# marja-w/gan-des-midi-music-gen

Hardware: AMD Instinct MI355X
Metric: GAN training samples/sec (G+D step) (higher is better)
Workload: dtype bf16; 1 GPU; SIMNN G/D iteration, synthetic 128x256 spectrogram windows; per_gpu_batch=256, global_batch=256, mode=faithful, parallelism=dp1

## Files before the change

### gan_des_midi_music_gen_amd/csrc/gemm_bf16.hip

```cpp
#include "gemm_common.h"

namespace {

constexpr int BM = 128, BN = 128;

inline bool operand_ok(const void* p, int dtype, int64_t s_row, int64_t s_k, int rows, int K, bool* kmaj) {
  const int64_t esz = dtype == GDM_BF16 ? 2 : 4, epc = 16 / esz;
  if (((uintptr_t)p & 15) != 0) return false;
  if (s_k == 1 && s_row >= 1 && (s_row * esz) % 16 == 0 && K % epc == 0) {
    *kmaj = true;
    return ((int64_t)(rows - 1) * s_row + K) * esz < ((int64_t)1 << 31);
  }
  if (s_row == 1 && s_k >= 1 && (s_k * esz) % 16 == 0 && rows % epc == 0) {
    *kmaj = false;
    return ((int64_t)(K - 1) * s_k + rows) * esz < ((int64_t)1 << 31);
  }
  return false;
}

}

bool gdm_gemm_bf16_fast_ok(const GemmArgs& g, int a_dtype, int b_dtype, bool* a_kmaj, bool* b_kmaj) {
  if (!operand_ok(g.A, a_dtype, g.sam, g.sak, g.M, g.K, a_kmaj)) return false;
  if (!operand_ok(g.B, b_dtype, g.sbn, g.sbk, g.N, g.K, b_kmaj)) return false;
  if (g.scn != 1) return false;
  const int64_t csz = g.c_dtype == GDM_BF16 ? 2 : 4;
  if (g.N % 4 == 0) {
    if ((g.scm * csz) % (4 * csz) != 0 || ((uintptr_t)g.C & (4 * csz - 1)) != 0) return false;
    if (g.bias_n && ((uintptr_t)g.bias_n & 15) != 0) return false;
  }
  if ((int64_t)g.M * g.N < 64 * 64) return false;
  return true;
}

bool gdm_gemm_bf16_fast_deep(int M, int N, int split_k, int k_per_split) {
  const int MT = (M + BM - 1) / BM, NTl = (N + BN - 1) / BN;
  const int outer = NTl * split_k;
  bool deep = split_k > 1 && (int64_t)outer * MT <= 512 && k_per_split >= 256;
  static const int force = GDM_TUNABLE("GDM_GEMM_VARIANT", -1);
  if (force >= 0) deep = force == 1;
  return deep;
}

int gdm_gemm_bf16_fast_launch(const GemmArgs& g, int a_dtype, int b_dtype, const GemmPlan& p, hipStream_t s) {
  const int MT = (g.M + BM - 1) / BM, NTl = (g.N + BN - 1) / BN;
  const int outer = NTl * g.split_k;
  dim3 grid((unsigned)(((outer + 7) / 8) * 8 * MT));
  const bool deep = p.kernel == GDM_GEMM_KERNEL_FAST_K64;
  auto* launch = a_dtype == GDM_BF16 ? (deep ? gdm_gemm_bf16_kt64_bf16a : gdm_gemm_bf16_kt32_bf16a)
                                     : (deep ? gdm_gemm_bf16_kt64_f32a : gdm_gemm_bf16_kt32_f32a);
  launch(g, p.a_kmaj, b_dtype, p.b_kmaj, grid, s);
  GDM_LAUNCH_OK("gdm_gemm(bf16 fast path)");
  return GDM_OK;
}
```

### gan_des_midi_music_gen_amd/csrc/gemm_bf16_kernel.h

```cpp
#pragma once
#include <type_traits>
#include "buffer_ops.h"
#include "gemm_common.h"

namespace {

constexpr int BM = 128, BN = 128, NT = 256;

__device__ __forceinline__ void wave_lds_sync() {
  __builtin_amdgcn_fence(__ATOMIC_RELEASE, "wavefront");
  __builtin_amdgcn_wave_barrier();
  __builtin_amdgcn_fence(__ATOMIC_ACQUIRE, "wavefront");
}

template <int ACT> __device__ __forceinline__ float act_const(float v, float slope) {
  if constexpr (ACT == GDM_ACT_RELU) return v > 0.f ? v : 0.f;
  else if constexpr (ACT == GDM_ACT_LEAKY) return v > 0.f ? v : v * slope;
  else if constexpr (ACT == GDM_ACT_SIGMOID) return 1.0f / (1.0f + expf(-v));
  else return v;
}

template <int KT> __device__ __forceinline__ int kswz(int row) { return KT == 64 ? ((row >> 1) & 7) : ((row >> 1) & 2); }
__device__ __forceinline__ int rswz(int k) { return (k & 3) | ((k >> 1) & 4); }

template <typename T, int KT> struct Stage {
  static constexpr int N = 128 * KT * (int)sizeof(T) / 16 / NT;
  f32x4 v[N];
};

template <typename T, int KT> struct Lane {
  uint32_t off[Stage<T, KT>::N];
  int kl[Stage<T, KT>::N];
  int lds[Stage<T, KT>::N];
};

template <typename T, int KT, bool KMAJ>
__device__ __forceinline__ void lane_init(Lane<T, KT>& ln, int64_t ld, int rows, int r0) {
  constexpr int EPC = 16 / sizeof(T);
  const int t = threadIdx.x;
#pragma unroll
  for (int i = 0; i < Stage<T, KT>::N; ++i) {
    const int c = t + NT * i;
    int rl, kl;
    if constexpr (KMAJ) {
      constexpr int CPR = KT / EPC;
      rl = c / CPR; kl = (c % CPR) * EPC;
      ln.off[i] = (uint32_t)(((int64_t)(r0 + rl) * ld + kl) * (int64_t)sizeof(T));
      ln.lds[i] = rl * KT + 8 * ((kl >> 3) ^ kswz<KT>(rl)) + (kl & 7);
    } else {
      constexpr int CPK = 128 / EPC;
      kl = c / CPK; rl = (c % CPK) * EPC;
      ln.off[i] = (uint32_t)(((int64_t)kl * ld + r0 + rl) * (int64_t)sizeof(T));
      ln.lds[i] = kl * 128 + (rl ^ (16 * rswz(kl)));
    }
    ln.kl[i] = (r0 + rl < rows) ? kl : -1;
  }
}

template <typename T, int KT, bool KMAJ>
__device__ __forceinline__ void stage_load(Stage<T, KT>& st, const Lane<T, KT>& ln, rsrc_t rs, int64_t ld, int k0,
                                           int kend) {
  const uint32_t kbytes = (uint32_t)((KMAJ ? (int64_t)k0 : (int64_t)k0 * ld) * (int64_t)sizeof(T));
#pragma unroll
  for (int i = 0; i < Stage<T, KT>::N; ++i) {
    const bool ok = ln.kl[i] >= 0 && k0 + ln.kl[i] < kend;
    st.v[i] = __builtin_bit_cast(f32x4, __builtin_amdgcn_raw_buffer_load_b128(rs, ok ? kbytes + ln.off[i] : BUF_OOB, 0, 0));
  }
}

template <typename T, int KT>
__device__ __forceinline__ void stage_store(const Stage<T, KT>& st, const Lane<T, KT>& ln, __bf16* __restrict__ img) {
#pragma unroll
  for (int i = 0; i < Stage<T, KT>::N; ++i) {
    if constexpr (sizeof(T) == 2) {
      *(f32x4*)(img + ln.lds[i]) = st.v[i];
    } else {
      bf16x4 h;
#pragma unroll
      for (int e = 0; e < 4; ++e) h[e] = (__bf16)st.v[i][e];
      *(bf16x4*)(img + ln.lds[i]) = h;
    }
  }
}

template <int KT, bool KMAJ>
__device__ __forceinline__ bf16x8 frag_read(const __bf16* __restrict__ img, int row0, int kk, int lr, int lg) {
  if constexpr (KMAJ) {
    const int row = row0 + lr;
    return *(const bf16x8*)&img[row * KT + 8 * ((4 * kk + lg) ^ kswz<KT>(row))];
  } else {
    const int q = lr >> 2, p = lr & 3;
    const int kr = 32 * kk + 8 * lg + q;
    const int n = (row0 + 4 * p) ^ (16 * (q | (4 * (lg & 1))));
    const bf16x4 lo = lds_tr16(&img[kr * 128 + n]);
    const bf16x4 hi = lds_tr16(&img[(kr + 4) * 128 + n]);
    return __builtin_shufflevector(lo, hi, 0, 1, 2, 3, 4, 5, 6, 7);
  }
}

template <typename TA, bool A_KMAJ, typename TB, bool B_KMAJ, int KT, int DEPTH>
__global__ __launch_bounds__(NT) void gemm_bf16_fast(GemmArgs g) {
  constexpr int IMG = 128 * KT;
  __shared__ __attribute__((aligned(16))) __bf16 smem[2 * DEPTH * IMG];
  const int t = threadIdx.x, l = t & 63, w = t >> 6, wm = w >> 1, wn = w & 1;
  const int lr = l & 15, lg = l >> 4;
  const int MT = (g.M + BM - 1) / BM, NTl = (g.N + BN - 1) / BN;
  const int id = blockIdx.x;
  const int grp = id / (8 * MT), within = id % (8 * MT);
  const int outer = grp * 8 + (within & 7), mt = within >> 3;
  if (outer >= NTl * g.split_k) return;
  const int nt = outer % NTl, zs = outer / NTl;
  const int m0 = mt * BM, n0 = nt * BN;
  const int kstep = KT * g.split_k;
  const int kbeg = zs * KT;
  const int kend = g.K;
  const int64_t lda = A_KMAJ ? g.sam : g.sak;
  const int64_t ldb = B_KMAJ ? g.sbn : g.sbk;
  const rsrc_t ra = make_rsrc(g.A, (uint32_t)((A_KMAJ ? (int64_t)(g.M - 1) * lda + g.K : (int64_t)(g.K - 1) * lda + g.M) *
                                             (int64_t)sizeof(TA)));
  const rsrc_t rb = make_rsrc(g.B, (uint32_t)((B_KMAJ ? (int64_t)(g.N - 1) * ldb + g.K : (int64_t)(g.K - 1) * ldb + g.N) *
                                             (int64_t)sizeof(TB)));
  Lane<TA, KT> la;
  Lane<TB, KT> lb;
  lane_init<TA, KT, A_KMAJ>(la, lda, g.M, m0);
  lane_init<TB, KT, B_KMAJ>(lb, ldb, g.N, n0);

  f32x4 acc[4][4];
#pragma unroll
  for (int i = 0; i < 4; ++i)
#pragma unroll
    for (int j = 0; j < 4; ++j) acc[i][j] = (f32x4){0.f, 0.f, 0.f, 0.f};

  auto multiply = [&](const __bf16* As, const __bf16* Bs) {
#pragma unroll
    for (int kk = 0; kk < KT / 32; ++kk) {
      bf16x8 a[4], b[4];
#pragma unroll
      for (int i = 0; i < 4; ++i) a[i] = frag_read<KT, A_KMAJ>(As, wm * 64 + 16 * i, kk, lr, lg);
#pragma unroll
      for (int j = 0; j < 4; ++j) b[j] = frag_read<KT, B_KMAJ>(Bs, wn * 64 + 16 * j, kk, lr, lg);
#pragma unroll
      for (int i = 0; i < 4; ++i)
#pragma unroll
        for (int j = 0; j < 4; ++j) acc[i][j] = mfma16(b[j], a[i], acc[i][j]);
    }
  };
  Stage<TA, KT> sa[DEPTH];
  Stage<TB, KT> sb[DEPTH];
  if constexpr (DEPTH == 2) {
    auto tile = [&](Stage<TA, KT>& xa, Stage<TB, KT>& xb, __bf16* As, int k0) {
      __bf16* Bs = As + IMG;
      stage_store<TA, KT>(xa, la, As);
      stage_store<TB, KT>(xb, lb, Bs);
      __syncthreads();
      stage_load<TA, KT, A_KMAJ>(xa, la, ra, lda, k0 + 2 * kstep, kend);
      stage_load<TB, KT, B_KMAJ>(xb, lb, rb, ldb, k0 + 2 * kstep, kend);
      multiply(As, Bs);
    };
    stage_load<TA, KT, A_KMAJ>(sa[0], la, ra, lda, kbeg, kend);
    stage_load<TB, KT, B_KMAJ>(sb[0], lb, rb, ldb, kbeg, kend);
    stage_load<TA, KT, A_KMAJ>(sa[1], la, ra, lda, kbeg + kstep, kend);
    stage_load<TB, KT, B_KMAJ>(sb[1], lb, rb, ldb, kbeg + kstep, kend);
    for (int k0 = kbeg; k0 < kend; k0 += 2 * kstep) {
      tile(sa[0], sb[0], smem, k0);
      tile(sa[DEPTH - 1], sb[DEPTH - 1], smem + 2 * IMG * (DEPTH - 1), k0 + kstep);
    }
  } else {
    __bf16* As = smem;
    __bf16* Bs = smem + IMG;
    stage_load<TA, KT, A_KMAJ>(sa[0], la, ra, lda, kbeg, kend);
    stage_load<TB, KT, B_KMAJ>(sb[0], lb, rb, ldb, kbeg, kend);
    for (int k0 = kbeg; k0 < kend; k0 += kstep) {
      __syncthreads();
      stage_store<TA, KT>(sa[0], la, As);
      stage_store<TB, KT>(sb[0], lb, Bs);
      __syncthreads();
      stage_load<TA, KT, A_KMAJ>(sa[0], la, ra, lda, k0 + kstep, kend);
      stage_load<TB, KT, B_KMAJ>(sb[0], lb, rb, ldb, k0 + kstep, kend);
      multiply(As, Bs);
    }
  }

  auto epilogue = [&](auto act_tag) {
    constexpr int ACT = decltype(act_tag)::value;
    const bool vec_ok = (g.N % 4 == 0);
    if (g.split_k > 1) {
#pragma unroll
      for (int i = 0; i < 4; ++i) {
        const int m = m0 + wm * 64 + 16 * i + lr;
        if (m >= g.M) continue;
#pragma unroll
        for (int j = 0; j < 4; ++j) {
          const int n = n0 + wn * 64 + 16 * j + 4 * lg;
          if (n >= g.N) continue;
          float* dst = g.ws + ((int64_t)zs * g.M + m) * g.N + n;
#ifndef GDM_GEMM_DEFAULT_STORES
          if (vec_ok) __builtin_nontemporal_store(acc[i][j], (f32x4*)dst);
#else
          if (vec_ok) *(f32x4*)dst = acc[i][j];
#endif
          else
            for (int r = 0; r < 4 && n + r < g.N; ++r) dst[r] = acc[i][j][r];
        }
      }
      return;
    }
    if (vec_ok && m0 + BM <= g.M && n0 + BN <= g.N &&
        (g.c_dtype != GDM_BF16 || (g.scm % 8 == 0 && ((uintptr_t)g.C & 15) == 0))) {
      __syncthreads();
      float* scr = (float*)smem + w * (16 * 64);
      const bool is_bf16 = g.c_dtype == GDM_BF16;
      const int prow = is_bf16 ? (l >> 3) : (l >> 4), pcol = is_bf16 ? 8 * (l & 7) : 4 * (l & 15);
      const int nn = n0 + wn * 64 + pcol;
      f32x4 bn0 = {0.f, 0.f, 0.f, 0.f}, bn1 = bn0;
      if (g.bias_n) {
        bn0 = *(const f32x4*)(g.bias_n + nn);
        if (is_bf16) bn1 = *(const f32x4*)(g.bias_n + nn + 4);
      }
      const bool has_bias = g.bias_n || g.bias_m;
#pragma unroll
      for (int i = 0; i < 4; ++i) {
        wave_lds_sync();
#pragma unroll
        for (int j = 0; j < 4; ++j) *(f32x4*)&scr[lr * 64 + 4 * ((4 * j + lg) ^ lr)] = acc[i][j];
        wave_lds_sync();
        if (is_bf16) {
#pragma unroll
          for (int h = 0; h < 2; ++h) {
            const int row = 8 * h + prow, c8 = l & 7;
            f32x4 v0 = *(const f32x4*)&scr[row * 64 + 4 * ((2 * c8) ^ row)];
            f32x4 v1 = *(const f32x4*)&scr[row * 64 + 4 * ((2 * c8 + 1) ^ row)];
            const int m = m0 + wm * 64 + 16 * i + row;
            if (has_bias) {
              const float bm = g.bias_m ? g.bias_m[m] : 0.f;
              v0 += bn0 + (f32x4){bm, bm, bm, bm};
              v1 += bn1 + (f32x4){bm, bm, bm, bm};
            }
            bf16x8 hv;
#pragma unroll
            for (int r = 0; r < 4; ++r) {
              hv[r] = (__bf16)act_const<ACT>(v0[r], g.slope);
              hv[4 + r] = (__bf16)act_const<ACT>(v1[r], g.slope);
            }
#ifndef GDM_GEMM_DEFAULT_STORES
            __builtin_nontemporal_store(hv, (bf16x8*)((__bf16*)g.C + (int64_t)m * g.scm + nn));
#else
            *(bf16x8*)((__bf16*)g.C + (int64_t)m * g.scm + nn) = hv;
#endif
          }
        } else {
#pragma unroll
          for (int h = 0; h < 4; ++h) {
            const int row = 4 * h + prow, pc = l & 15;
            f32x4 v = *(const f32x4*)&scr[row * 64 + 4 * (pc ^ row)];
            const int m = m0 + wm * 64 + 16 * i + row;
            if (has_bias) {
              const float bm = g.bias_m ? g.bias_m[m] : 0.f;
              v += bn0 + (f32x4){bm, bm, bm, bm};
            }
#pragma unroll
            for (int r = 0; r < 4; ++r) v[r] = act_const<ACT>(v[r], g.slope);
#ifndef GDM_GEMM_DEFAULT_STORES
            __builtin_nontemporal_store(v, (f32x4*)((float*)g.C + (int64_t)m * g.scm + nn));
#else
            *(f32x4*)((float*)g.C + (int64_t)m * g.scm + nn) = v;
#endif
          }
        }
      }
      return;
    }
#pragma unroll
    for (int i = 0; i < 4; ++i) {
      const int m = m0 + wm * 64 + 16 * i + lr;
      if (m >= g.M) continue;
#pragma unroll
      for (int j = 0; j < 4; ++j) {
        const int n = n0 + wn * 64 + 16 * j + 4 * lg;
        if (n >= g.N) continue;
        f32x4 v = acc[i][j];
        for (int r = 0; r < 4 && n + r < g.N; ++r) {
          float y = v[r];
          if (g.bias_n) y += g.bias_n[n + r];
          if (g.bias_m) y += g.bias_m[m];
          store_from_f32(g.C, g.c_dtype, (int64_t)m * g.scm + n + r, act_const<ACT>(y, g.slope));
        }
      }
    }
  };
  switch (g.act) {
    case GDM_ACT_RELU: epilogue(std::integral_constant<int, GDM_ACT_RELU>{}); break;
    case GDM_ACT_LEAKY: epilogue(std::integral_constant<int, GDM_ACT_LEAKY>{}); break;
    case GDM_ACT_SIGMOID: epilogue(std::integral_constant<int, GDM_ACT_SIGMOID>{}); break;
    default: epilogue(std::integral_constant<int, GDM_ACT_NONE>{}); break;
  }
}

template <typename TA, int KT, int DEPTH, bool AK, typename TB>
void launch_b(const GemmArgs& g, bool b_kmaj, dim3 grid, hipStream_t s) {
  if (b_kmaj) hipLaunchKernelGGL((gemm_bf16_fast<TA, AK, TB, true, KT, DEPTH>), grid, dim3(NT), 0, s, g);
  else hipLaunchKernelGGL((gemm_bf16_fast<TA, AK, TB, false, KT, DEPTH>), grid, dim3(NT), 0, s, g);
}
template <typename TA, int KT, int DEPTH, bool AK>
void launch_a(const GemmArgs& g, int b_dtype, bool b_kmaj, dim3 grid, hipStream_t s) {
  if (b_dtype == GDM_BF16) launch_b<TA, KT, DEPTH, AK, __bf16>(g, b_kmaj, grid, s);
  else launch_b<TA, KT, DEPTH, AK, float>(g, b_kmaj, grid, s);
}
template <typename TA, int KT, int DEPTH>
void launch_instances(const GemmArgs& g, bool a_kmaj, int b_dtype, bool b_kmaj, dim3 grid, hipStream_t s) {
  if (a_kmaj) launch_a<TA, KT, DEPTH, true>(g, b_dtype, b_kmaj, grid, s);
  else launch_a<TA, KT, DEPTH, false>(g, b_dtype, b_kmaj, grid, s);
}

}
```

### gan_des_midi_music_gen_amd/csrc/gemm_bf16_kt32_bf16a.hip

```cpp
#include "gemm_bf16_kernel.h"

void gdm_gemm_bf16_kt32_bf16a(const GemmArgs& g, bool a_kmaj, int b_dtype, bool b_kmaj, dim3 grid, hipStream_t s) {
  launch_instances<__bf16, 32, 1>(g, a_kmaj, b_dtype, b_kmaj, grid, s);
}
```

### gan_des_midi_music_gen_amd/csrc/gemm_bf16_kt32_f32a.hip

```cpp
#include "gemm_bf16_kernel.h"

void gdm_gemm_bf16_kt32_f32a(const GemmArgs& g, bool a_kmaj, int b_dtype, bool b_kmaj, dim3 grid, hipStream_t s) {
  launch_instances<float, 32, 1>(g, a_kmaj, b_dtype, b_kmaj, grid, s);
}
```

### gan_des_midi_music_gen_amd/csrc/gemm_bf16_kt64_bf16a.hip

```cpp
#include "gemm_bf16_kernel.h"

void gdm_gemm_bf16_kt64_bf16a(const GemmArgs& g, bool a_kmaj, int b_dtype, bool b_kmaj, dim3 grid, hipStream_t s) {
  launch_instances<__bf16, 64, 2>(g, a_kmaj, b_dtype, b_kmaj, grid, s);
}
```

### gan_des_midi_music_gen_amd/csrc/gemm_bf16_kt64_f32a.hip

```cpp
#include "gemm_bf16_kernel.h"

void gdm_gemm_bf16_kt64_f32a(const GemmArgs& g, bool a_kmaj, int b_dtype, bool b_kmaj, dim3 grid, hipStream_t s) {
  launch_instances<float, 64, 2>(g, a_kmaj, b_dtype, b_kmaj, grid, s);
}
```

### gan_des_midi_music_gen_amd/csrc/gemm_common.h

```cpp
#pragma once
#include "gdm_common.h"

struct GemmArgs {
  const void* A; int64_t sam, sak;
  const void* B; int64_t sbk, sbn;
  void* C; int c_dtype; int64_t scm, scn;
  int M, N, K;
  const float* bias_n; const float* bias_m; int act; float slope;
  int split_k, k_per_split; float* ws;
};

__device__ __forceinline__ void gemm_epilogue_store(const GemmArgs& g, int m, int n, float v) {
  if (g.bias_n) v += g.bias_n[n];
  if (g.bias_m) v += g.bias_m[m];
  v = apply_act(v, g.act, g.slope);
  store_from_f32(g.C, g.c_dtype, (int64_t)m * g.scm + (int64_t)n * g.scn, v);
}

struct GemmPlan {
  int kernel;
  bool a_kmaj, b_kmaj;
  int split_k, k_per_split;
  int reduce;
  size_t ws_bytes;
};

bool gdm_gemm_bf16_fast_ok(const GemmArgs& g, int a_dtype, int b_dtype, bool* a_kmaj, bool* b_kmaj);
bool gdm_gemm_bf16_fast_deep(int M, int N, int split_k, int k_per_split);
int gdm_gemm_bf16_fast_launch(const GemmArgs& g, int a_dtype, int b_dtype, const GemmPlan& p, hipStream_t s);
void gdm_gemm_bf16_kt32_bf16a(const GemmArgs& g, bool a_kmaj, int b_dtype, bool b_kmaj, dim3 grid, hipStream_t s);
void gdm_gemm_bf16_kt32_f32a(const GemmArgs& g, bool a_kmaj, int b_dtype, bool b_kmaj, dim3 grid, hipStream_t s);
void gdm_gemm_bf16_kt64_bf16a(const GemmArgs& g, bool a_kmaj, int b_dtype, bool b_kmaj, dim3 grid, hipStream_t s);
void gdm_gemm_bf16_kt64_f32a(const GemmArgs& g, bool a_kmaj, int b_dtype, bool b_kmaj, dim3 grid, hipStream_t s);
constexpr int GDM_GEMM_FAST_KT = 64;
```

Measured before the change: 444,200 samples/s.

## Generalize bf16 GEMM prefetch into register ring with scheduler pinning

Replaces the fixed DEPTH 1/2 staging in the bf16 fast GEMM with a configurable register ring of prefetched tiles, decoupled from the LDS buffer count. When both operands are bf16 and the K loop is long enough, the KT32 path now prefetches two tiles ahead instead of one. Ring variants also insert sched_barrier pins so the compiler cannot reorder global loads past the MFMA block. The aim is to hide global-load latency, at the cost of extra registers and more template instances.

```diff
diff --git a/gan_des_midi_music_gen_amd/csrc/gemm_bf16.hip b/gan_des_midi_music_gen_amd/csrc/gemm_bf16.hip
--- a/gan_des_midi_music_gen_amd/csrc/gemm_bf16.hip
+++ b/gan_des_midi_music_gen_amd/csrc/gemm_bf16.hip
@@ -47,9 +47,19 @@
   const int outer = NTl * g.split_k;
   dim3 grid((unsigned)(((outer + 7) / 8) * 8 * MT));
   const bool deep = p.kernel == GDM_GEMM_KERNEL_FAST_K64;
-  auto* launch = a_dtype == GDM_BF16 ? (deep ? gdm_gemm_bf16_kt64_bf16a : gdm_gemm_bf16_kt32_bf16a)
-                                     : (deep ? gdm_gemm_bf16_kt64_f32a : gdm_gemm_bf16_kt32_f32a);
-  launch(g, p.a_kmaj, b_dtype, p.b_kmaj, grid, s);
+  const bool both_bf16 = a_dtype == GDM_BF16 && b_dtype == GDM_BF16;
+  const int kt = deep ? 64 : 32;
+  const int tiles = ((g.K + kt - 1) / kt + g.split_k - 1) / g.split_k;
+  if (both_bf16 && deep) {
+    gdm_gemm_bf16_ring_kt64(g, p.a_kmaj, p.b_kmaj, grid, s);
+  } else if (both_bf16 && tiles >= GDM_GEMM_RING_K32) {
+    gdm_gemm_bf16_ring_kt32(g, p.a_kmaj, p.b_kmaj, grid, s);
+  } else if (a_dtype == GDM_BF16 && deep) {
+    gdm_gemm_bf16_kt64_bf16a_f32b(g, p.a_kmaj, p.b_kmaj, grid, s);
+  } else {
+    auto* launch = a_dtype == GDM_BF16 ? gdm_gemm_bf16_kt32_bf16a : (deep ? gdm_gemm_bf16_kt64_f32a : gdm_gemm_bf16_kt32_f32a);
+    launch(g, p.a_kmaj, b_dtype, p.b_kmaj, grid, s);
+  }
   GDM_LAUNCH_OK("gdm_gemm(bf16 fast path)");
   return GDM_OK;
 }
diff --git a/gan_des_midi_music_gen_amd/csrc/gemm_bf16_kernel.h b/gan_des_midi_music_gen_amd/csrc/gemm_bf16_kernel.h
--- a/gan_des_midi_music_gen_amd/csrc/gemm_bf16_kernel.h
+++ b/gan_des_midi_music_gen_amd/csrc/gemm_bf16_kernel.h
@@ -98,10 +98,12 @@
   }
 }
 
-template <typename TA, bool A_KMAJ, typename TB, bool B_KMAJ, int KT, int DEPTH>
+template <typename TA, bool A_KMAJ, typename TB, bool B_KMAJ, int KT, int RING, bool PIN>
 __global__ __launch_bounds__(NT) void gemm_bf16_fast(GemmArgs g) {
   constexpr int IMG = 128 * KT;
-  __shared__ __attribute__((aligned(16))) __bf16 smem[2 * DEPTH * IMG];
+  constexpr int NBUF = KT == 64 ? 2 : 1;
+  constexpr int UNROLL = RING % NBUF == 0 ? RING : RING * NBUF;
+  __shared__ __attribute__((aligned(16))) __bf16 smem[2 * NBUF * IMG];
   const int t = threadIdx.x, l = t & 63, w = t >> 6, wm = w >> 1, wn = w & 1;
   const int lr = l & 15, lg = l >> 4;
   const int MT = (g.M + BM - 1) / BM, NTl = (g.N + BN - 1) / BN;
@@ -145,38 +147,31 @@
         for (int j = 0; j < 4; ++j) acc[i][j] = mfma16(b[j], a[i], acc[i][j]);
     }
   };
-  Stage<TA, KT> sa[DEPTH];
-  Stage<TB, KT> sb[DEPTH];
-  if constexpr (DEPTH == 2) {
-    auto tile = [&](Stage<TA, KT>& xa, Stage<TB, KT>& xb, __bf16* As, int k0) {
+  Stage<TA, KT> sa[RING];
+  Stage<TB, KT> sb[RING];
+  auto pin = [] {
+    if constexpr (PIN) __builtin_amdgcn_sched_barrier(0);
+  };
+#pragma unroll
+  for (int r = 0; r < RING; ++r) {
+    stage_load<TA, KT, A_KMAJ>(sa[r], la, ra, lda, kbeg + r * kstep, kend);
+    stage_load<TB, KT, B_KMAJ>(sb[r], lb, rb, ldb, kbeg + r * kstep, kend);
+    pin();
+  }
+  for (int k0 = kbeg; k0 < kend; k0 += UNROLL * kstep) {
+#pragma unroll
+    for (int u = 0; u < UNROLL; ++u) {
+      Stage<TA, KT>& xa = sa[u % RING];
+      Stage<TB, KT>& xb = sb[u % RING];
+      __bf16* As = smem + 2 * IMG * (u % NBUF);
       __bf16* Bs = As + IMG;
+      if constexpr (NBUF == 1) __syncthreads();
       stage_store<TA, KT>(xa, la, As);
       stage_store<TB, KT>(xb, lb, Bs);
       __syncthreads();
-      stage_load<TA, KT, A_KMAJ>(xa, la, ra, lda, k0 + 2 * kstep, kend);
-      stage_load<TB, KT, B_KMAJ>(xb, lb, rb, ldb, k0 + 2 * kstep, kend);
-      multiply(As, Bs);
-    };
-    stage_load<TA, KT, A_KMAJ>(sa[0], la, ra, lda, kbeg, kend);
-    stage_load<TB, KT, B_KMAJ>(sb[0], lb, rb, ldb, kbeg, kend);
-    stage_load<TA, KT, A_KMAJ>(sa[1], la, ra, lda, kbeg + kstep, kend);
-    stage_load<TB, KT, B_KMAJ>(sb[1], lb, rb, ldb, kbeg + kstep, kend);
-    for (int k0 = kbeg; k0 < kend; k0 += 2 * kstep) {
-      tile(sa[0], sb[0], smem, k0);
-      tile(sa[DEPTH - 1], sb[DEPTH - 1], smem + 2 * IMG * (DEPTH - 1), k0 + kstep);
-    }
-  } else {
-    __bf16* As = smem;
-    __bf16* Bs = smem + IMG;
-    stage_load<TA, KT, A_KMAJ>(sa[0], la, ra, lda, kbeg, kend);
-    stage_load<TB, KT, B_KMAJ>(sb[0], lb, rb, ldb, kbeg, kend);
-    for (int k0 = kbeg; k0 < kend; k0 += kstep) {
-      __syncthreads();
-      stage_store<TA, KT>(sa[0], la, As);
-      stage_store<TB, KT>(sb[0], lb, Bs);
-      __syncthreads();
-      stage_load<TA, KT, A_KMAJ>(sa[0], la, ra, lda, k0 + kstep, kend);
-      stage_load<TB, KT, B_KMAJ>(sb[0], lb, rb, ldb, k0 + kstep, kend);
+      stage_load<TA, KT, A_KMAJ>(xa, la, ra, lda, k0 + (u + RING) * kstep, kend);
+      stage_load<TB, KT, B_KMAJ>(xb, lb, rb, ldb, k0 + (u + RING) * kstep, kend);
+      pin();
       multiply(As, Bs);
     }
   }
@@ -296,20 +291,15 @@
   }
 }
 
-template <typename TA, int KT, int DEPTH, bool AK, typename TB>
-void launch_b(const GemmArgs& g, bool b_kmaj, dim3 grid, hipStream_t s) {
-  if (b_kmaj) hipLaunchKernelGGL((gemm_bf16_fast<TA, AK, TB, true, KT, DEPTH>), grid, dim3(NT), 0, s, g);
-  else hipLaunchKernelGGL((gemm_bf16_fast<TA, AK, TB, false, KT, DEPTH>), grid, dim3(NT), 0, s, g);
-}
-template <typename TA, int KT, int DEPTH, bool AK>
-void launch_a(const GemmArgs& g, int b_dtype, bool b_kmaj, dim3 grid, hipStream_t s) {
-  if (b_dtype == GDM_BF16) launch_b<TA, KT, DEPTH, AK, __bf16>(g, b_kmaj, grid, s);
-  else launch_b<TA, KT, DEPTH, AK, float>(g, b_kmaj, grid, s);
-}
-template <typename TA, int KT, int DEPTH>
-void launch_instances(const GemmArgs& g, bool a_kmaj, int b_dtype, bool b_kmaj, dim3 grid, hipStream_t s) {
-  if (a_kmaj) launch_a<TA, KT, DEPTH, true>(g, b_dtype, b_kmaj, grid, s);
-  else launch_a<TA, KT, DEPTH, false>(g, b_dtype, b_kmaj, grid, s);
-}
-
-}
+template <typename TA, typename TB, int KT, int RING, bool PIN>
+void launch_layouts(const GemmArgs& g, bool a_kmaj, bool b_kmaj, dim3 grid, hipStream_t s) {
+  if (a_kmaj) {
+    if (b_kmaj) hipLaunchKernelGGL((gemm_bf16_fast<TA, true, TB, true, KT, RING, PIN>), grid, dim3(NT), 0, s, g);
+    else hipLaunchKernelGGL((gemm_bf16_fast<TA, true, TB, false, KT, RING, PIN>), grid, dim3(NT), 0, s, g);
+  } else {
+    if (b_kmaj) hipLaunchKernelGGL((gemm_bf16_fast<TA, false, TB, true, KT, RING, PIN>), grid, dim3(NT), 0, s, g);
+    else hipLaunchKernelGGL((gemm_bf16_fast<TA, false, TB, false, KT, RING, PIN>), grid, dim3(NT), 0, s, g);
+  }
+}
+
+}
diff --git a/gan_des_midi_music_gen_amd/csrc/gemm_bf16_kt32_bf16a.hip b/gan_des_midi_music_gen_amd/csrc/gemm_bf16_kt32_bf16a.hip
--- a/gan_des_midi_music_gen_amd/csrc/gemm_bf16_kt32_bf16a.hip
+++ b/gan_des_midi_music_gen_amd/csrc/gemm_bf16_kt32_bf16a.hip
@@ -1,5 +1,6 @@
 #include "gemm_bf16_kernel.h"
 
 void gdm_gemm_bf16_kt32_bf16a(const GemmArgs& g, bool a_kmaj, int b_dtype, bool b_kmaj, dim3 grid, hipStream_t s) {
-  launch_instances<__bf16, 32, 1>(g, a_kmaj, b_dtype, b_kmaj, grid, s);
+  if (b_dtype == GDM_BF16) launch_layouts<__bf16, __bf16, 32, 1, false>(g, a_kmaj, b_kmaj, grid, s);
+  else launch_layouts<__bf16, float, 32, 1, false>(g, a_kmaj, b_kmaj, grid, s);
 }
diff --git a/gan_des_midi_music_gen_amd/csrc/gemm_bf16_kt32_f32a.hip b/gan_des_midi_music_gen_amd/csrc/gemm_bf16_kt32_f32a.hip
--- a/gan_des_midi_music_gen_amd/csrc/gemm_bf16_kt32_f32a.hip
+++ b/gan_des_midi_music_gen_amd/csrc/gemm_bf16_kt32_f32a.hip
@@ -1,5 +1,6 @@
 #include "gemm_bf16_kernel.h"
 
 void gdm_gemm_bf16_kt32_f32a(const GemmArgs& g, bool a_kmaj, int b_dtype, bool b_kmaj, dim3 grid, hipStream_t s) {
-  launch_instances<float, 32, 1>(g, a_kmaj, b_dtype, b_kmaj, grid, s);
+  if (b_dtype == GDM_BF16) launch_layouts<float, __bf16, 32, 1, false>(g, a_kmaj, b_kmaj, grid, s);
+  else launch_layouts<float, float, 32, 1, false>(g, a_kmaj, b_kmaj, grid, s);
 }
diff --git a/gan_des_midi_music_gen_amd/csrc/gemm_bf16_kt64_bf16a.hip b/gan_des_midi_music_gen_amd/csrc/gemm_bf16_kt64_bf16a.hip
--- a/gan_des_midi_music_gen_amd/csrc/gemm_bf16_kt64_bf16a.hip
+++ b/gan_des_midi_music_gen_amd/csrc/gemm_bf16_kt64_bf16a.hip
@@ -1,5 +1,5 @@
 #include "gemm_bf16_kernel.h"
 
-void gdm_gemm_bf16_kt64_bf16a(const GemmArgs& g, bool a_kmaj, int b_dtype, bool b_kmaj, dim3 grid, hipStream_t s) {
-  launch_instances<__bf16, 64, 2>(g, a_kmaj, b_dtype, b_kmaj, grid, s);
+void gdm_gemm_bf16_kt64_bf16a_f32b(const GemmArgs& g, bool a_kmaj, bool b_kmaj, dim3 grid, hipStream_t s) {
+  launch_layouts<__bf16, float, 64, 2, false>(g, a_kmaj, b_kmaj, grid, s);
 }
diff --git a/gan_des_midi_music_gen_amd/csrc/gemm_bf16_kt64_f32a.hip b/gan_des_midi_music_gen_amd/csrc/gemm_bf16_kt64_f32a.hip
--- a/gan_des_midi_music_gen_amd/csrc/gemm_bf16_kt64_f32a.hip
+++ b/gan_des_midi_music_gen_amd/csrc/gemm_bf16_kt64_f32a.hip
@@ -1,5 +1,6 @@
 #include "gemm_bf16_kernel.h"
 
 void gdm_gemm_bf16_kt64_f32a(const GemmArgs& g, bool a_kmaj, int b_dtype, bool b_kmaj, dim3 grid, hipStream_t s) {
-  launch_instances<float, 64, 2>(g, a_kmaj, b_dtype, b_kmaj, grid, s);
+  if (b_dtype == GDM_BF16) launch_layouts<float, __bf16, 64, 2, false>(g, a_kmaj, b_kmaj, grid, s);
+  else launch_layouts<float, float, 64, 2, false>(g, a_kmaj, b_kmaj, grid, s);
 }
diff --git a/gan_des_midi_music_gen_amd/csrc/gemm_bf16_ring_kt32.hip b/gan_des_midi_music_gen_amd/csrc/gemm_bf16_ring_kt32.hip
--- /dev/null
+++ b/gan_des_midi_music_gen_amd/csrc/gemm_bf16_ring_kt32.hip
@@ -0,0 +1,5 @@
+#include "gemm_bf16_kernel.h"
+
+void gdm_gemm_bf16_ring_kt32(const GemmArgs& g, bool a_kmaj, bool b_kmaj, dim3 grid, hipStream_t s) {
+  launch_layouts<__bf16, __bf16, 32, GDM_GEMM_RING_K32, true>(g, a_kmaj, b_kmaj, grid, s);
+}
diff --git a/gan_des_midi_music_gen_amd/csrc/gemm_bf16_ring_kt64.hip b/gan_des_midi_music_gen_amd/csrc/gemm_bf16_ring_kt64.hip
--- /dev/null
+++ b/gan_des_midi_music_gen_amd/csrc/gemm_bf16_ring_kt64.hip
@@ -0,0 +1,5 @@
+#include "gemm_bf16_kernel.h"
+
+void gdm_gemm_bf16_ring_kt64(const GemmArgs& g, bool a_kmaj, bool b_kmaj, dim3 grid, hipStream_t s) {
+  launch_layouts<__bf16, __bf16, 64, GDM_GEMM_RING_K64, true>(g, a_kmaj, b_kmaj, grid, s);
+}
diff --git a/gan_des_midi_music_gen_amd/csrc/gemm_common.h b/gan_des_midi_music_gen_amd/csrc/gemm_common.h
--- a/gan_des_midi_music_gen_amd/csrc/gemm_common.h
+++ b/gan_des_midi_music_gen_amd/csrc/gemm_common.h
@@ -30,6 +30,14 @@
 int gdm_gemm_bf16_fast_launch(const GemmArgs& g, int a_dtype, int b_dtype, const GemmPlan& p, hipStream_t s);
 void gdm_gemm_bf16_kt32_bf16a(const GemmArgs& g, bool a_kmaj, int b_dtype, bool b_kmaj, dim3 grid, hipStream_t s);
 void gdm_gemm_bf16_kt32_f32a(const GemmArgs& g, bool a_kmaj, int b_dtype, bool b_kmaj, dim3 grid, hipStream_t s);
-void gdm_gemm_bf16_kt64_bf16a(const GemmArgs& g, bool a_kmaj, int b_dtype, bool b_kmaj, dim3 grid, hipStream_t s);
+void gdm_gemm_bf16_kt64_bf16a_f32b(const GemmArgs& g, bool a_kmaj, bool b_kmaj, dim3 grid, hipStream_t s);
 void gdm_gemm_bf16_kt64_f32a(const GemmArgs& g, bool a_kmaj, int b_dtype, bool b_kmaj, dim3 grid, hipStream_t s);
+void gdm_gemm_bf16_ring_kt32(const GemmArgs& g, bool a_kmaj, bool b_kmaj, dim3 grid, hipStream_t s);
+void gdm_gemm_bf16_ring_kt64(const GemmArgs& g, bool a_kmaj, bool b_kmaj, dim3 grid, hipStream_t s);
+#ifndef GDM_GEMM_RING_K64
+#define GDM_GEMM_RING_K64 2
+#endif
+#ifndef GDM_GEMM_RING_K32
+#define GDM_GEMM_RING_K32 2
+#endif
 constexpr int GDM_GEMM_FAST_KT = 64;
```

Result: faster. 448,700 samples/s (median of 6 runs) (+1.0%).
